# edshkim98/LocalDiffusion-Hallucination

Hardware: AMD Instinct MI355X
Metric: local patches/sec (256^2, T=1000) (higher is better)
Workload: dtype bf16; 1 GPU; cfg3: 8 local patches (vertical band masks) of one 3x256x256 image per GPU, 4-stage dim-32 conditional UNet (12.1M params), DDPM T=1000, pred_x0, sigmoid schedule; patches_per_gpu=8, parallelism=patch-sharded x1, one all-gather per sample, step_graph_replay=True, whole_batch_graph_flag=False, concurrent_sub_batches=2, weight_split_levels=0

## Files before the change

include/localdiff_hip.h:

```cpp
#ifndef LOCALDIFF_HIP_H
#define LOCALDIFF_HIP_H

#include <stddef.h>
#include <stdint.h>

#ifdef __cplusplus
extern "C" {
#endif

#define LD_OK 0
#define LD_EINVAL (-1)
#define LD_EHIP (-2)
#define LD_ETIMEOUT (-3)

#define LD_F32 0
#define LD_BF16 1
#define LD_F16 2

#define LD_STAT_STRIPES 16

#define LD_ACT_NONE 0
#define LD_ACT_SILU 1
#define LD_ACT_RELU 2

// ... 125 lines not shown

int ld_linattn_kmax(const void* qkv, uint32_t* kmax_enc, int B, int n, int heads, int dim_head,
                    int dtype, void* stream);
int ld_linattn_ctx(const void* qkv, const uint32_t* kmax_enc, float* ctx_part,
                   int B, int n, int heads, int dim_head, int nchunks, int dtype, void* stream);
int ld_linattn_ctx_reduce(const float* ctx_part, int nchunks, float* ctxn, int B, int heads,
                          int dim_head, void* stream);
int ld_linattn_fold(const float* ctxn, const float* w_out ,
                    void* w_packed , int B, int C, int heads, int dim_head,
                    int perm, int dtype, void* stream);
int ld_linattn_ctxfold(const float* ctx_part, int nchunks, const float* w_out ,
                       void* w_packed , int B, int C, int heads, int dim_head,
                       int perm, int dtype, void* stream);
int ld_linattn_kvctx(const void* x, const void* wkv_packed, const float* kshift, float* ctx_part, int B,
                     int n, int C, int heads, int dim_head, int nchunks, int dtype, void* stream);
int ld_linattn_out(const void* x, const void* wq_packed, const float* qshift, const void* mfold,
                   const float* bias, const float* g2, void* out, int B, int n, int C, float q_scale,
                   int dtype, void* stream);
int ld_linattn_kvctx_terms(const void* x, const void* wkv_packed, const float* kshift, float* ctx_part, int B, int n, int C,
                           int heads, int dim_head, int nchunks, int dtype, int weight_terms, void* stream);
int ld_linattn_out_terms(const void* x, const void* wq_packed, const float* qshift, const void* mfold, const float* bias,
                         const float* g2, void* out, int B, int n, int C, float q_scale, int dtype, int weight_terms,
                         void* stream);
size_t ld_linattn_ctx_part_floats(int B, int heads, int dim_head, int nchunks);

int ld_attention(const void* qkv, void* out, int B, int n, int heads, int dim_head, int dtype,
                 void* stream);

int ld_time_mlp(const int32_t* times, int n, const float* freqs, int dim, const float* w1,
                const float* b1, const float* w2, const float* b2, int time_dim, float* temb,
                void* stream);
int ld_time_mlp_fourier(const int32_t* times, int n, const float* weights, int learned_dim, const float* w1,
                        const float* b1, const float* w2, const float* b2, int time_dim, float* temb, void* stream);
int ld_film(const float* temb, int n, int time_dim, const float* w, const float* b, int two_c,
            float* film, void* stream);

int ld_final_conv(const void* x, const float* w , const float* b, float* out_nchw,
                  int B, int H, int W, int Cin, int Cout, int dtype, void* stream);

int ld_final_step(const void* x, const float* w, const float* b, float* model_out, float* x_t, float* x0_out,
                  const float* sched, const int32_t* t_ptr, float lo, float hi, int objective, uint64_t seed,
                  int64_t noise_stream, int B, int H, int W, int Cin, int Cout, int dtype, void* stream);


int ld_final_step_at(const void* x, const float* w, const float* b, float* model_out, float* x_t, float* x0_out,
                     const float* sched, const int32_t* t_ptr, float lo, float hi, int objective, uint64_t seed,
// ... 141 lines not shown
```

localdiffusion-hallucination_amd/_cabi.py:

```python
import ctypes as C
import os

from .tuning import lib_override_path

_HERE = os.path.dirname(os.path.abspath(__file__))

LIB_PATH = lib_override_path() or os.path.join(_HERE, "csrc", "liblocaldiff_hip.so")

LD_F32, LD_BF16, LD_F16 = 0, 1, 2
ACT_NONE, ACT_SILU, ACT_RELU = 0, 1, 2
EPI_PLAIN, EPI_QKV_LINEAR, EPI_QKV_FULL, EPI_RMS_RES, EPI_RES, EPI_GN_TAIL = 0, 1, 2, 3, 4, 5
OBJ = {"pred_x0": 0, "pred_noise": 1, "pred_v": 2}
SCHED_COLS = 8
STAT_STRIPES = 16
COUNTER_CONV3X3_C32, COUNTER_CONV3X3_GENERIC, COUNTER_CONV3X3_S32 = 0, 1, 2
SEG_SRC_PLAIN, SEG_SRC_POOL, SEG_SRC_CAT_D2S = 0, 1, 2

vp, i32, i64, u64, f32 = C.c_void_p, C.c_int32, C.c_int64, C.c_uint64, C.c_float


class Src(C.Structure):
    _fields_ = [("data", vp), ("C", i32), ("pix_stride", i32), ("upsample", i32), ("gn_stats", vp),
                ("gn_gamma", vp), ("gn_beta", vp), ("gn_groups", i32), ("act", i32), ("film", vp),
                ("film_tstride", i32), ("film_bstride", i32)]
# ... 57 lines not shown
    "ld_tuning_name": (C.c_char_p, [C.c_int]),
    "ld_range_push": (C.c_int, [C.c_char_p]),
    "ld_range_pop": (C.c_int, []),
    "ld_conv3x3": (C.c_int, [C.POINTER(Conv3x3Args), vp]),
    "ld_conv1x1": (C.c_int, [C.POINTER(Conv1x1Args), vp]),
    "ld_pack_conv_weight": (C.c_int, [vp, vp, vp, C.c_int, C.c_int, C.c_int, C.c_int, C.c_int, vp]),
    "ld_pack_conv_weight_terms": (C.c_int, [vp, vp, vp, C.c_int, C.c_int, C.c_int, C.c_int, C.c_int, C.c_int, vp]),
    "ld_conv_image": (C.c_int, [vp, vp, vp, vp, vp, C.c_int, C.c_int, C.c_int, C.c_int, C.c_int,
                                C.c_int, C.c_int, vp]),
    "ld_stem_packed_bytes": (C.c_size_t, []),
    "ld_pack_stem_weight": (C.c_int, [vp, vp, C.c_int, vp]),
    "ld_conv_stem": (C.c_int, [vp, vp, vp, vp, C.c_int, C.c_int, C.c_int, C.c_int, C.c_int, vp]),
    "ld_conv_stem_begin": (C.c_int, [vp, vp, vp, vp, C.c_int, C.c_int, C.c_int, C.c_int, C.c_int, C.POINTER(StepBeginArgs), vp]),
    "ld_gn_apply": (C.c_int, [C.POINTER(GnApplyArgs), vp]),
    "ld_linattn_kmax": (C.c_int, [vp, vp, C.c_int, C.c_int, C.c_int, C.c_int, C.c_int, vp]),
    "ld_linattn_ctx": (C.c_int, [vp, vp, vp, C.c_int, C.c_int, C.c_int, C.c_int, C.c_int, C.c_int, vp]),
    "ld_linattn_ctx_reduce": (C.c_int, [vp, C.c_int, vp, C.c_int, C.c_int, C.c_int, vp]),
    "ld_linattn_fold": (C.c_int, [vp, vp, vp, C.c_int, C.c_int, C.c_int, C.c_int, C.c_int, C.c_int, vp]),
    "ld_linattn_ctxfold": (C.c_int, [vp, C.c_int, vp, vp, C.c_int, C.c_int, C.c_int, C.c_int, C.c_int, C.c_int, vp]),
    "ld_linattn_kvctx": (C.c_int, [vp, vp, vp, vp, C.c_int, C.c_int, C.c_int, C.c_int, C.c_int, C.c_int, C.c_int, vp]),
    "ld_linattn_out": (C.c_int, [vp, vp, vp, vp, vp, vp, vp, C.c_int, C.c_int, C.c_int, f32, C.c_int, vp]),
    "ld_linattn_kvctx_terms": (C.c_int, [vp, vp, vp, vp, C.c_int, C.c_int, C.c_int, C.c_int, C.c_int, C.c_int, C.c_int, C.c_int, vp]),
    "ld_linattn_out_terms": (C.c_int, [vp, vp, vp, vp, vp, vp, vp, C.c_int, C.c_int, C.c_int, f32, C.c_int, C.c_int, vp]),
    "ld_linattn_ctx_part_floats": (C.c_size_t, [C.c_int, C.c_int, C.c_int, C.c_int]),
    "ld_attention": (C.c_int, [vp, vp, C.c_int, C.c_int, C.c_int, C.c_int, C.c_int, vp]),
    "ld_time_mlp": (C.c_int, [vp, C.c_int, vp, C.c_int, vp, vp, vp, vp, C.c_int, vp, vp]),
    "ld_time_mlp_fourier": (C.c_int, [vp, C.c_int, vp, C.c_int, vp, vp, vp, vp, C.c_int, vp, vp]),
    "ld_film": (C.c_int, [vp, C.c_int, C.c_int, vp, vp, C.c_int, vp, vp]),
    "ld_final_conv": (C.c_int, [vp, vp, vp, vp, C.c_int, C.c_int, C.c_int, C.c_int, C.c_int, C.c_int, vp]),
    "ld_final_step": (C.c_int, [vp, vp, vp, vp, vp, vp, vp, vp, f32, f32, C.c_int, u64, i64, C.c_int, C.c_int, C.c_int,
                                C.c_int, C.c_int, C.c_int, vp]),
    "ld_final_step_at": (C.c_int, [vp, vp, vp, vp, vp, vp, vp, vp, f32, f32, C.c_int, u64, i64, i64, i64, vp, C.c_int,
                                   C.c_int, C.c_int, C.c_int, C.c_int, C.c_int, vp]),
    "ld_timing_begin": (C.c_int, [C.c_int]),
    "ld_timing_count": (C.c_int, []),
    "ld_timing_end": (C.c_int, [vp, C.c_int, vp]),
    "ld_timing_end_abs": (C.c_int, [vp, vp, C.c_int, vp]),
    "ld_randn": (C.c_int, [vp, i64, u64, i64, i64, vp, vp]),
    "ld_randn_at": (C.c_int, [vp, i64, i64, u64, i64, i64, vp, vp]),
    "ld_step_add": (C.c_int, [vp, C.c_int, vp]),
    "ld_step_begin": (C.c_int, [vp, C.c_size_t, vp, C.c_size_t, vp, C.c_int, vp, vp, vp]),
    "ld_step_begin_film": (C.c_int, [vp, C.c_size_t, vp, C.c_size_t, vp, C.c_int, vp, vp, vp, C.c_int, vp, vp]),
    "ld_ddim_step_at": (C.c_int, [vp, vp, vp, vp, vp, vp, f32, f32, C.c_int, i64, vp]),
    "ld_ddpm_step": (C.c_int, [vp, vp, vp, vp, vp, vp, vp, f32, f32, C.c_int, i64, vp]),
    "ld_posterior_step": (C.c_int, [vp, vp, vp, vp, vp, vp, i64, vp]),
    "ld_ddim_step": (C.c_int, [vp, vp, vp, vp, f32, f32, f32, f32, f32, f32, f32, f32, f32, C.c_int,
# ... 95 lines not shown
```

localdiffusion-hallucination_amd/csrc/linattn_fused.hip:

```cpp
#include "common.hip.h"
#include <stdlib.h>

typedef __attribute__((ext_vector_type(4))) short s16x4;

namespace {
constexpr int CTX_STRIDE = 32 * 32 + 64;
constexpr int KTN = 256;
constexpr int PROW = 96;

__device__ __forceinline__ uint2 tr8(const char* p) {
  s16x4 v = __builtin_amdgcn_ds_read_tr16_b64_v4i16((__attribute__((address_space(3))) s16x4*)(const_cast<char*>(p)));
  return __builtin_bit_cast(uint2, v);
}

struct KvCtxArgs {
  const void* x;
  const uint4* wkv;
  float* ctx_part;
  int n, C, heads, nchunks;
  const float* kshift;
  int wsplit;
};
#define KVCTX_PARAMS const void* x_, const uint4* wkv_, float* ctx_part_, int n_, int C_, int heads_, int nchunks_, const float* kshift_, int wsplit_
#define KVCTX_ARGS(a) (a).x, (a).wkv, (a).ctx_part, (a).n, (a).C, (a).heads, (a).nchunks, (a).kshift, (a).wsplit
// ... 137 lines not shown
        }
    }
  }
  float* dst = a.ctx_part + (((size_t)b * a.heads + h) * a.nchunks + ck) * CTX_STRIDE;
#pragma unroll
  for (int r = 0; r < 4; ++r) store_f32_out(&dst[(dt * 16 + kq * 4 + r) * 32 + et * 16 + li], cacc[r]);
  __syncthreads();
  float* s_z = reinterpret_cast<float*>(s_p);
#pragma unroll
  for (int m = 0; m < 2; ++m)
#pragma unroll
    for (int r = 0; r < 4; ++r) {
      const float z = wave16_sum(zs[m][r]);
      if (li == 0) s_z[wv * 32 + 16 * m + 4 * kq + r] = z;
    }
  __syncthreads();
  if (tid < 32) {
    store_f32_out(&dst[1024 + tid], s_z[tid] + s_z[32 + tid] + s_z[64 + tid] + s_z[96 + tid]);
    store_f32_out(&dst[1056 + tid], fmaxf(fmaxf(s_m[tid], s_m[32 + tid]), fmaxf(s_m[64 + tid], s_m[96 + tid])));
  }
}


template <typename T, int NCH, bool SINGLE, int WS = 0>
__global__ __launch_bounds__(256) void kvctx_wph_kernel(KVCTX_PARAMS) {
  const KvCtxArgs a{x_, wkv_, ctx_part_, n_, C_, heads_, nchunks_, kshift_, wsplit_};
  constexpr int NCW = NCH << WS;
  constexpr int PLANE = KTN * 16;
  extern __shared__ __attribute__((aligned(16))) char smem[];
  char* s_x = smem;
  float* s_rinv = reinterpret_cast<float*>(s_x + NCH * 4 * PLANE);
  const int ck = blockIdx.x, b = blockIdx.y;
  const int tid = threadIdx.x, lane = tid & 63, wv = tid >> 6, li = lane & 15, kq = lane >> 4;
  const int h = wv;
  const int n = a.n, C = a.C;
  const int npc = (n + a.nchunks - 1) / a.nchunks;
  const int lo = ck * npc, hi = min(n, lo + npc);
  uint4 A[4][NCW];
#pragma unroll
  for (int c = 0; c < NCW; ++c)
#pragma unroll
    for (int m = 0; m < 4; ++m) A[m][c] = a.wkv[(((size_t)h * NCW + c) * 4 + m) * 64 + lane];
  float cmax[2], mloc[2], zs[2];
#pragma unroll
  for (int m = 0; m < 2; ++m) { cmax[m] = -INFINITY; mloc[m] = 0.f; zs[m] = 0.f; }
  f32x4 cacc[2][2];
#pragma unroll
  for (int i = 0; i < 2; ++i)
#pragma unroll
    for (int j = 0; j < 2; ++j) cacc[i][j] = f32x4{0.f, 0.f, 0.f, 0.f};
  const T* xb = reinterpret_cast<const T*>(a.x) + (size_t)b * n * C;

  uint4 xr[NCH][4];
  auto issue = [&](int p0) {
#pragma unroll
    for (int c = 0; c < NCH; ++c)
#pragma unroll
      for (int it = 0; it < 4; ++it) {
        const int p = p0 + (it * 4 + wv) * 16 + li;
        xr[c][it] = make_uint4(0u, 0u, 0u, 0u);
        if (p < hi) xr[c][it] = *reinterpret_cast<const uint4*>(xb + (size_t)p * C + c * 32 + kq * 8);
      }
  };
  issue(lo);
  constexpr int first_pass = SINGLE ? 1 : 0;
  if (SINGLE) {
#pragma unroll
    for (int m = 0; m < 2; ++m) mloc[m] = a.kshift[h * 32 + 16 * m + li];
  }
  constexpr float LOG2E = 1.4426950408889634f;
  float m2[2];
#pragma unroll
  for (int m = 0; m < 2; ++m) m2[m] = mloc[m] * LOG2E - DT<T>::pshift;
  for (int pass = first_pass; pass < 2; ++pass) {
    for (int p0 = lo; p0 < hi; p0 += KTN) {
      __syncthreads();
      float rs[4] = {0.f, 0.f, 0.f, 0.f};
#pragma unroll
      for (int c = 0; c < NCH; ++c)
#pragma unroll
        for (int it = 0; it < 4; ++it) {
          const int qq = (it * 4 + wv) * 16 + li;
          const uint4 raw = xr[c][it];
          float v[8];
          unpack16<T>(raw, v);
#pragma unroll
          for (int e = 0; e < 8; ++e) rs[it] = fmaf(v[e], v[e], rs[it]);
          *reinterpret_cast<uint4*>(s_x + (c * 4 + kq) * PLANE + qq * 16) = raw;
        }
#pragma unroll
      for (int it = 0; it < 4; ++it) {
        float r = rs[it];
        r = kq4_sum(r);
        if (kq == 0) s_rinv[(it * 4 + wv) * 16 + li] = rms_rinv<false>(r);
      }
      __syncthreads();
      {
        const int nxt = p0 + KTN;
        if (nxt < hi) issue(nxt);
// ... 69 lines not shown
        }
      }
    }
    if (!SINGLE && pass == 0) {
#pragma unroll
      for (int m = 0; m < 2; ++m) { mloc[m] = kq4_max(cmax[m]); m2[m] = mloc[m] * LOG2E - DT<T>::pshift; }
    }
  }
  float* dst = a.ctx_part + (((size_t)b * a.heads + h) * a.nchunks + ck) * CTX_STRIDE;
#pragma unroll
  for (int dt = 0; dt < 2; ++dt)
#pragma unroll
    for (int et = 0; et < 2; ++et)
#pragma unroll
      for (int r = 0; r < 4; ++r) store_f32_out(&dst[(dt * 16 + kq * 4 + r) * 32 + et * 16 + li], cacc[dt][et][r]);
#pragma unroll
  for (int m = 0; m < 2; ++m) {
    const float z = kq4_sum(zs[m]);
    if (kq == 0) {
      store_f32_out(&dst[1024 + 16 * m + li], z);
      store_f32_out(&dst[1056 + 16 * m + li], mloc[m]);
    }
  }
}

constexpr int LINOUT_TPB = 1;

struct LinOutArgs {
  const void* x;
  const uint4* wq;
  const uint4* mfold;
  const float* bias;
  const float* g2;
  void* out;
  int n, C;
  float q_scale;
  const float* qshift;
  int wsplit;
};
#define LINOUT_PARAMS const void* x_, const uint4* wq_, const uint4* mfold_, const float* bias_, const float* g2_, const float* qshift_, \
                      int n_, int C_, void* out_, float q_scale_, int wsplit_
#define LINOUT_ARGS(a) (a).x, (a).wq, (a).mfold, (a).bias, (a).g2, (a).qshift, (a).n, (a).C, (a).out, (a).q_scale, (a).wsplit

template <typename T, int NCH, int WS = 0>
__global__ __launch_bounds__(256) void linout_kernel(LINOUT_PARAMS) {
  const LinOutArgs a{x_, wq_, mfold_, bias_, g2_, out_, n_, C_, q_scale_, qshift_, wsplit_};
// ... 184 lines not shown
      if (kshift) LD_LAUNCH((kvctx_wph_kernel<T, 4, true>), grid2, dim3(256), lds2, st, KVCTX_ARGS(a));
      else LD_LAUNCH((kvctx_wph_kernel<T, 4, false>), grid2, dim3(256), lds2, st, KVCTX_ARGS(a));
    }
    LD_LAUNCH_CHECK("linattn_kvctx(wave-per-head)");
    return LD_OK;
  }
  LD_REQUIRE(!a.wsplit, "ld_linattn_kvctx: two-term weights need heads == 4 (the wave-per-head kernel)");
  dim3 grid(nchunks, heads, B);
  const size_t lds = (size_t)nch * 4 * KTN * 16 + 2 * KTN * PROW + KTN * sizeof(float) + 128 * sizeof(float);
  if (nch == 1) {
    LD_LAUNCH((kvctx_kernel<T, 1>), grid, dim3(256), lds, st, KVCTX_ARGS(a));
  } else if (nch == 2) {
    LD_HIP(ld_allow_lds((kvctx_kernel<T, 2>), lds));
    LD_LAUNCH((kvctx_kernel<T, 2>), grid, dim3(256), lds, st, KVCTX_ARGS(a));
  } else {
    LD_HIP(ld_allow_lds((kvctx_kernel<T, 4>), lds));
    LD_LAUNCH((kvctx_kernel<T, 4>), grid, dim3(256), lds, st, KVCTX_ARGS(a));
  }
  LD_LAUNCH_CHECK("linattn_kvctx");
  return LD_OK;
}

template <typename T>
int linout_launch(const LinOutArgs& a, int B, hipStream_t st) {
  const int n = a.n, nch = a.C / 32;
  dim3 grid((n + 128 * LINOUT_TPB - 1) / (128 * LINOUT_TPB), B);
  const size_t lds = (size_t)nch * 4 * 128 * 16 + ((size_t)nch << a.wsplit) * 8 * 1024 + (size_t)4 * 2 * nch * 1024 + 128 * sizeof(float);
  if (a.wsplit) {
    LD_REQUIRE(nch <= 2, "ld_linattn_out: two-term weights are built for C = 32 / 64 (got %d)", a.C);
    if (nch == 1) LD_LAUNCH((linout_kernel<T, 1, 1>), grid, dim3(256), lds, st, LINOUT_ARGS(a));
    else LD_LAUNCH((linout_kernel<T, 2, 1>), grid, dim3(256), lds, st, LINOUT_ARGS(a));
  } else if (nch == 1) {
    LD_LAUNCH((linout_kernel<T, 1>), grid, dim3(256), lds, st, LINOUT_ARGS(a));
  } else if (nch == 2) {
    LD_LAUNCH((linout_kernel<T, 2>), grid, dim3(256), lds, st, LINOUT_ARGS(a));
  } else {
    LD_HIP(ld_allow_lds((linout_kernel<T, 4>), lds));
    LD_LAUNCH((linout_kernel<T, 4>), grid, dim3(256), lds, st, LINOUT_ARGS(a));
  }
  LD_LAUNCH_CHECK("linattn_out");
  return LD_OK;
}
}

extern "C" int ld_linattn_kvctx(const void* x, const void* wkv_packed, const float* kshift, float* ctx_part, int B,
                                int n, int C, int heads, int dim_head, int nchunks, int dtype, void* stream) {
  return ld_linattn_kvctx_terms(x, wkv_packed, kshift, ctx_part, B, n, C, heads, dim_head, nchunks, dtype, 1, stream);
}

extern "C" int ld_linattn_kvctx_terms(const void* x, const void* wkv_packed, const float* kshift, float* ctx_part, int B,
                                      int n, int C, int heads, int dim_head, int nchunks, int dtype, int weight_terms,
                                      void* stream) {
  LD_REQUIRE(weight_terms == 1 || weight_terms == 2, "ld_linattn_kvctx: weight_terms %d", weight_terms);
  LD_REQUIRE(x && wkv_packed && ctx_part && B > 0 && n > 0 && nchunks > 0, "ld_linattn_kvctx: bad args");
  LD_REQUIRE(ld_dtype_16(dtype), "ld_linattn_kvctx: 16-bit storage only (fp32 uses the unfused path)");
  LD_REQUIRE(dim_head == 32 && (C == 32 || C == 64 || C == 128), "ld_linattn_kvctx: dim_head 32, C in {32,64,128}");
  LD_REQUIRE(kshift == nullptr || heads == 4, "ld_linattn_kvctx: the single-sweep mode (kshift) needs heads == 4");
  KvCtxArgs a{x, (const uint4*)wkv_packed, ctx_part, n, C, heads, nchunks, kshift, weight_terms == 2 ? 1 : 0};
  hipStream_t st = reinterpret_cast<hipStream_t>(stream);
  return LD_DISPATCH16(dtype, kvctx_launch<T>(a, B, st));
}

extern "C" int ld_linattn_out(const void* x, const void* wq_packed, const float* qshift, const void* mfold,
                              const float* bias, const float* g2, void* out, int B, int n, int C, float q_scale,
                              int dtype, void* stream) {
  return ld_linattn_out_terms(x, wq_packed, qshift, mfold, bias, g2, out, B, n, C, q_scale, dtype, 1, stream);
}

extern "C" int ld_linattn_out_terms(const void* x, const void* wq_packed, const float* qshift, const void* mfold,
                                    const float* bias, const float* g2, void* out, int B, int n, int C, float q_scale,
                                    int dtype, int weight_terms, void* stream) {
  LD_REQUIRE(weight_terms == 1 || weight_terms == 2, "ld_linattn_out: weight_terms %d", weight_terms);
  LD_REQUIRE(x && wq_packed && mfold && bias && g2 && out && B > 0 && n > 0, "ld_linattn_out: bad args");
  LD_REQUIRE(ld_dtype_16(dtype), "ld_linattn_out: 16-bit storage only (fp32 uses the unfused path)");
  LD_REQUIRE(C == 32 || C == 64 || C == 128, "ld_linattn_out: C in {32,64,128}");
  LinOutArgs a{x, (const uint4*)wq_packed, (const uint4*)mfold, bias, g2, out, n, C, q_scale, qshift, weight_terms == 2 ? 1 : 0};
  return LD_DISPATCH16(dtype, linout_launch<T>(a, B, reinterpret_cast<hipStream_t>(stream)));
}
```

localdiffusion-hallucination_amd/unet.py:

```python
import ctypes as C
import math

import numpy as np
import torch
from torch import nn

from . import _cabi as cabi
from .pool import check_declared, intervals_from_declared, peak_live, place_intervals
from .tuning import Tuning
from .weights import UnetConfig, unet_param_shapes

_TORCH_DT = {"fp32": torch.float32, "bf16": torch.bfloat16, "fp16": torch.float16}
_LOWP = ("bf16", "fp16")


def _register(root: nn.Module, dotted: str, tensor: torch.Tensor):
    parts = dotted.split(".")
    mod = root
    for name in parts[:-1]:
        if name not in mod._modules:
            mod.add_module(name, nn.Module())
        mod = mod._modules[name]
    mod.register_parameter(parts[-1], nn.Parameter(tensor, requires_grad=False))

# ... 191 lines not shown
                    part = part.contiguous()
                    out = torch.empty(part.numel(), dtype=tdt, device=dev)
                    cabi.check(lib.ld_pack_conv_weight(part.data_ptr(), None, out.data_ptr(), part.shape[0], part.shape[1],
                                                       k, 0, dt, st), "pack " + nm + tag)
                    P["w"][nm + tag] = out
                    P.setdefault("keep", []).append(part)
        if self.compute_dtype in _LOWP and self.cfg.init_dim == 32:
            wi = sd["init_conv.weight"].contiguous()
            stem = torch.empty(int(lib.ld_stem_packed_bytes()), dtype=torch.uint8, device=dev)
            cabi.check(lib.ld_pack_stem_weight(wi.data_ptr(), stem.data_ptr(), wi.shape[1], st), "pack init_conv")
            P["stem"] = stem
            P.setdefault("keep", []).append(wi)
        for name, w in sd.items():
            if name.endswith(".to_out.1.g"):
                g = w.flatten()
                P["g2"][name] = (g * math.sqrt(g.numel())).contiguous()
        half = self.cfg.dim // 2
        step = math.log(self.theta) / (half - 1)
        P["freqs"] = torch.exp(torch.arange(half) * -step).to(dev)
        torch.cuda.current_stream().synchronize()
        self._packed, self._packed_key = P, key
        return P

    def plan(self, B, H, W, table_T=None, instance=0):
        f = self.downsample_factor
        assert H % f == 0 and W % f == 0, \
            f"your input dimensions {(H, W)} need to be divisible by {f}, given the unet"
        tn = self.tuning
        key = (B, H, W, table_T, self.compute_dtype, instance, self.weight_split_levels,
               tn.separate_act, tn.sep_act_max_px, tn.sep_act_min_c, tn.fusion_fold, tn.side_res_conv, tn.side_res_conv_max_px, tn.side_res_conv_px, tn.fused_step_begin, tn.linattn_chunk_px, tn.buffer_reuse, tn.recompute_stem, tn.pool_by_size, tn.pool_verify)
        if key not in self._plans:
            self._plans[key] = _Plan(self, B, H, W, table_T)
        return self._plans[key]

    @torch.no_grad()
    def forward(self, x, cond_img, time, x_self_cond=None):
        B, _, H, W = x.shape
        if self.self_condition:
            c = self.cfg.channels
            raise RuntimeError(f"Given groups=1, weight of size [{self.cfg.init_dim}, {c}, 7, 7], expected input[{B}, {2 * c}, {H}, {W}] to have "
                               f"{c} channels, but got {2 * c} channels instead (self_condition=True: ddpm.py:406-413)")
        p = self.plan(B, H, W)
        st = torch.cuda.current_stream().cuda_stream
        p.x_in.copy_(x.to(torch.float32))
        p.cond_in.copy_(cond_img.to(torch.float32))
        p.times.copy_(time.to(torch.int32))
        p.run_time(st)
        p.run_cond(st)
        p.run_main(st)
        return p.model_out.clone()


class _Plan:

    def __init__(self, net: Unet, B, H, W, table_T=None):
        self.net, self.B, self.H, self.W, self.table_T = net, B, H, W, table_T
        self.lib = cabi.lib()
        self.dev = net.device
        self.dt = cabi.dtype_code(net.compute_dtype)
        self.tdt = _TORCH_DT[net.compute_dtype]
        self.esize = 4 if self.dt == cabi.LD_F32 else 2
        self.P = net.packed()
        self.tn = net.tuning
        self.f32 = self.P["f32"]
        cfg = net.cfg
        self.cfg = cfg
        self.keep = []
        self._track = None
        self.named = {}
        self.meta = {}
        self.decl = {}
        self.live_out = []
        self.ops_time, self.ops_cond, self.ops_main = [], [], []
        self.nslot = 0
        self.stats = torch.zeros(160, B, cabi.STAT_STRIPES, 16, 2, dtype=torch.float64, device=self.dev)
        self.cond_slots = 16
        self.kmax_arena = torch.zeros(8, B, cabi.STAT_STRIPES, cfg.hidden, dtype=torch.int32, device=self.dev)
        self._kmax_cursor = 0
        self.x_in = torch.zeros(B, cfg.channels, H, W, dtype=torch.float32, device=self.dev)
# ... 342 lines not shown
        if cfg.learned_sinusoidal_dim:
            wts = f["time_mlp.0.weights"]
            self.ops_time.append(lambda st: cabi.check(lib.ld_time_mlp_fourier(
                times.data_ptr(), n, wts.data_ptr(), cfg.learned_sinusoidal_dim, f["time_mlp.1.weight"].data_ptr(),
                f["time_mlp.1.bias"].data_ptr(), f["time_mlp.3.weight"].data_ptr(), f["time_mlp.3.bias"].data_ptr(),
                td, self.temb.data_ptr(), st), "time_mlp (learned Fourier features)"))
        else:
            self.ops_time.append(lambda st: cabi.check(lib.ld_time_mlp(
                times.data_ptr(), n, freqs.data_ptr(), cfg.dim, f["time_mlp.1.weight"].data_ptr(),
                f["time_mlp.1.bias"].data_ptr(), f["time_mlp.3.weight"].data_ptr(), f["time_mlp.3.bias"].data_ptr(),
                td, self.temb.data_ptr(), st), "time_mlp"))
        for name in f:
            if name.endswith(".mlp.1.weight") and not name.startswith("conv_fusion"):
                p = name[:-len(".mlp.1.weight")]
                two_c = f[name].shape[0]
                film = torch.zeros(n, two_c, dtype=torch.float32, device=self.dev)
                self.films[p] = film
                self._film_off[id(film)] = self.film_row
                self.film_row += two_c
                w, b = f[name], f[p + ".mlp.1.bias"]
                self.ops_time.append(lambda st, w=w, b=b, film=film, two_c=two_c: cabi.check(lib.ld_film(
                    self.temb.data_ptr(), n, td, w.data_ptr(), b.data_ptr(), two_c, film.data_ptr(), st), "film"))

    def resnet_block(self, ops, p, srcs_fn, cin_total, cout, h, w, res_tensor=None):
        f, G = self.f32, self.cfg.resnet_block_groups
        s1, s2 = self.slot(), self.slot()
        wres = self.P["w"].get(p + ".res_conv.weight")
        side = None
        px_ok = (h * w in self.tn.side_res_conv_px) if self.tn.side_res_conv_px is not None else h * w <= self.tn.side_res_conv_max_px
        if (wres is not None and self.tn.side_res_conv and self.dt != cabi.LD_F32 and px_ok and self.net.weight_split_levels == 0
                and wres.data_ptr() not in self.P["terms2"] and self.P["w"][p + ".block1.proj.weight"].data_ptr() not in self.P["terms2"]):
            side = (wres, f[p + ".res_conv.bias"])
        rc = None
        if side is not None:
            raw1, rc = self.conv3(ops, srcs_fn(), p + ".block1.proj", cout, h, w, stats=s1, groups=G, side=side)
        else:
            raw1 = self.conv3(ops, srcs_fn(), p + ".block1.proj", cout, h, w, stats=s1, groups=G)
        film = self.films.get(p)
        n1 = self.src(raw1, cout, gn=(s1, f[p + ".block1.norm.weight"], f[p + ".block1.norm.bias"], G),
                      act=cabi.ACT_SILU, film=film)
        if self._separate_act(h * w, cout):
            act1 = self.gn_apply(ops, n1, None, h, w, cout)
            n1 = self.src(act1, cout)
        raw2 = self.conv3(ops, [n1], p + ".block2.proj", cout, h, w, stats=s2, groups=G)
        n2 = self.src(raw2, cout, gn=(s2, f[p + ".block2.norm.weight"], f[p + ".block2.norm.bias"], G),
                      act=cabi.ACT_SILU)
        if rc is not None:
            out = self.gn_apply(ops, n2, self.src(rc, cout), h, w, cout)
        elif (p + ".res_conv.weight") in f:
            out = self.conv1(ops, srcs_fn(), self.P["w"][p + ".res_conv.weight"], cout, h, w,
                             bias=f[p + ".res_conv.bias"], epi=cabi.EPI_GN_TAIL, gn_tail=n2, what="res_conv+tail " + p)
        else:
            assert res_tensor is not None and cin_total == cout
            out = self.gn_apply(ops, n2, self.src(res_tensor, cout), h, w, cout)
        self.named[p] = out
        return out

    def fusion_block_folded(self, ops, x, c, h, w):
        f, G, p = self.f32, self.cfg.resnet_block_groups, "conv_fusion"
        p1, p2, zero = self.fusion_const
        s1, s2 = self.slot(), self.slot()
        raw1 = self.conv3(ops, [self.src(x, c)], p + ".block1.proj", c, h, w, stats=s1, groups=G,
                          weight=self.P["w"][p + ".block1.proj.weight#x"], bias=zero, addend=p1)
        n1 = self.src(raw1, c, gn=(s1, f[p + ".block1.norm.weight"], f[p + ".block1.norm.bias"], G),
                      act=cabi.ACT_SILU, film=self.films.get(p))
        if self._separate_act(h * w, c):
            n1 = self.src(self.gn_apply(ops, n1, None, h, w, c), c)
        raw2 = self.conv3(ops, [n1], p + ".block2.proj", c, h, w, stats=s2, groups=G)
        n2 = self.src(raw2, c, gn=(s2, f[p + ".block2.norm.weight"], f[p + ".block2.norm.bias"], G), act=cabi.ACT_SILU)
        out = self.conv1(ops, [self.src(x, c)], self.P["w"][p + ".res_conv.weight#x"], c, h, w, bias=None,
                         epi=cabi.EPI_GN_TAIL, gn_tail=n2, residual=p2, what="res_conv+tail " + p)
        self.named[p] = out
        return out

    def linear_attention_fused(self, ops, p, x, c, h, w):
        f, cfg, lib = self.f32, self.cfg, self.lib
        n, hid, B, heads, dt, es = h * w, cfg.hidden, self.B, cfg.attn_heads, self.dt, self.esize
        rule = self.tn.chunk_rule(B)
        chunk_px = rule[0] if n >= 65536 else (rule[1] if n >= 16384 else rule[2])
        nchunks = max(1, min(128, n // chunk_px)) if heads == 4 else max(1, min(32, n // 256))
        if heads == 4 and self.tn.linattn_chunk_px is None:
            while B * nchunks < 512 and nchunks < 512 and n // (2 * nchunks) >= 256:
                nchunks *= 2
        ctx = self._tracked(torch.empty(int(lib.ld_linattn_ctx_part_floats(B, heads, 32, nchunks)), dtype=torch.float32, device=self.dev))
        wfold = self._tracked(torch.empty(B, c * hid, dtype=self.tdt, device=self.dev))
        wout = f[p + ".to_out.0.weight"].reshape(c, hid).contiguous()
        wq, wkv = self.P["wq"][p], self.P["wkv"][p]
        kshift = self.P["kshift"].get(p) if heads == 4 else None
        ksp = kshift.data_ptr() if kshift is not None else None
        qshift = self.P["qshift"].get(p) if heads == 4 else None
        qsp = qshift.data_ptr() if qshift is not None else None
        bias, g2 = f[p + ".to_out.0.bias"], self.P["g2"][p + ".to_out.1.g"]
        out = self.buf(h, w, c)
        self.keep += [ctx, wfold, wout, wq, wkv, kshift, qshift, bias, g2, out, x]
        npx = B * n
        terms = self.P.get("attn_terms", {}).get(p, 1)
        self._raw(ops, lambda st: cabi.check(lib.ld_linattn_kvctx_terms(x.data_ptr(), wkv.data_ptr(), ksp, ctx.data_ptr(), B, n, c,
                                                                        heads, 32, nchunks, dt, terms, st), "linattn_kvctx"),
                  "linattn_kvctx", nbytes=npx * c * es, flops=2 * npx * c * 2 * hid * (1 if kshift is not None else 2) + 2 * npx * hid * 32,
                  reads=[x], writes=[ctx])
        self._raw(ops, lambda st: cabi.check(lib.ld_linattn_ctxfold(ctx.data_ptr(), nchunks, wout.data_ptr(), wfold.data_ptr(), B, c,
                                                                    heads, 32, 1, dt, st), "linattn_ctxfold"),
                  "linattn_ctxfold", nbytes=B * c * hid * es, flops=2 * B * c * hid * 32, reads=[ctx], writes=[wfold])
        scale = cfg.attn_dim_head ** -0.5
        self._raw(ops, lambda st: cabi.check(lib.ld_linattn_out_terms(x.data_ptr(), wq.data_ptr(), qsp, wfold.data_ptr(), bias.data_ptr(),
                                                                      g2.data_ptr(), out.data_ptr(), B, n, c, scale, dt, terms, st),
                                             "linattn_out"),
                  "linattn_out", nbytes=2 * npx * c * es, flops=2 * npx * hid * c * 2, reads=[x, wfold], writes=[out])
        return out

    def linear_attention(self, ops, p, x, c, h, w):
        if self.dt != cabi.LD_F32 and c in (32, 64, 128) and p in self.P["wq"]:
            return self.linear_attention_fused(ops, p, x, c, h, w)
        f, cfg, lib = self.f32, self.cfg, self.lib
        n, hid, B = h * w, cfg.hidden, self.B
        kmax = self.kmax_arena[self._kmax_cursor]
        self._kmax_cursor += 1
        qkv = self.conv1(ops, [self.src(x, c)], self.P["w"][p + ".to_qkv.weight"], 3 * hid, h, w,
                         epi=cabi.EPI_QKV_LINEAR, rms_in=1, what="to_qkv " + p, kmax_out=kmax)
        nchunks = max(1, min(32, n // 256))
        ctx = torch.empty(int(lib.ld_linattn_ctx_part_floats(B, cfg.attn_heads, 32, nchunks)),
                          dtype=torch.float32, device=self.dev)
        wfold = torch.empty(B, c * hid, dtype=self.tdt, device=self.dev)
# ... 8 lines not shown
                                                                    B, c, heads, 32, 0, dt, st), "linattn_ctxfold"),
                  "linattn_ctxfold", nbytes=B * c * hid * es, flops=2 * B * c * hid * 32, reads=[ctx], writes=[wfold])
        q = self.src(qkv, hid, stride=3 * hid)
        return self.conv1(ops, [q], wfold, c, h, w, bias=f[p + ".to_out.0.bias"], epi=cabi.EPI_RMS_RES,
                          bstride=c * hid * self.esize, g2=self.P["g2"][p + ".to_out.1.g"], residual=x,
                          what="lin to_out " + p)

    def full_attention(self, ops, p, x, c, h, w):
        f, cfg, lib = self.f32, self.cfg, self.lib
        n, hid, B = h * w, cfg.hidden, self.B
        qkv = self.conv1(ops, [self.src(x, c)], self.P["w"][p + ".to_qkv.weight"], 3 * hid, h, w,
                         epi=cabi.EPI_QKV_FULL, rms_in=1, what="to_qkv " + p)
        att = self.buf(h, w, hid)
        dt, heads = self.dt, cfg.attn_heads
        self.keep += [qkv, att]
        self._raw(ops, lambda st: cabi.check(lib.ld_attention(qkv.data_ptr(), att.data_ptr(), B, n, heads, 32, dt, st),
                                             "attention"),
                  "attention", nbytes=4 * B * n * hid * self.esize, flops=4 * B * n * n * hid, reads=[qkv], writes=[att])
        return self.conv1(ops, [self.src(att, hid)], self.P["w"][p + ".to_out.weight"], c, h, w,
                          bias=f[p + ".to_out.bias"], epi=cabi.EPI_RES, residual=x, what="full to_out " + p)

    def attention(self, ops, p, x, c, h, w, full):
        out = (self.full_attention if full else self.linear_attention)(ops, p, x, c, h, w)
        self.named[p] = out
        return out

    def _basic_block(self, ops, p, x, cin, cmid, cout, h, w, pool, image=False):
        f, lib, G = self.f32, self.lib, 16
        s1, s2, s3 = self.slot(), self.slot(), self.slot()

        def image_conv(wname, c_out, stats):
            out = self.buf(h, w, c_out)
            wt, bs = f[wname + ".weight"], f[wname + ".bias"]
            B, dt = self.B, self.dt
            self.keep += [out, wt, bs]
            ops.append(lambda st: cabi.check(lib.ld_conv_image(
                self.cond_in.data_ptr(), wt.data_ptr(), bs.data_ptr(), out.data_ptr(), stats.data_ptr(), G,
                B, cin, h, w, 3, dt, st), "conv_image " + wname))
            return out

        if image:
            a1 = image_conv(p + ".convblock.0", cmid, s1)
            idr = image_conv(p + ".identity.0", cout, s3)
        else:
            a1 = self.conv3(ops, [self.src(x, cin)], p + ".convblock.0", cmid, h, w, stats=s1, groups=G)
            idr = self.conv3(ops, [self.src(x, cin)], p + ".identity.0", cout, h, w, stats=s3, groups=G)
# ... 28 lines not shown
                za, ba, zb, bb = self._begin_args
                rows, row_floats, cur = self._film_args
                g = cabi.StepBeginArgs(za, ba, zb, bb, self._t_dev_ptr, int(delta), idx_ptr, t_table, rows, row_floats, cur)
                cabi.check(lib.ld_conv_stem_begin(self.x_in.data_ptr(), wstem.data_ptr(), bi.data_ptr(), r.data_ptr(), B, cfg.channels,
                                                  H, W, self.dt, C.byref(g), st), "init_conv + step_begin")
            self._stem_begin = stem_begin
            self._raw(ops, lambda st: cabi.check(lib.ld_conv_stem(
                self.x_in.data_ptr(), wstem.data_ptr(), bi.data_ptr(), r.data_ptr(), B, cfg.channels, H, W, self.dt, st),
                "init_conv"), "conv_image7x7",
                nbytes=B * H * W * (4 * cfg.channels + self.esize * cfg.init_dim), flops=2 * 49 * cfg.channels * cfg.init_dim * B * H * W, writes=[r])
        else:
            self._raw(ops, lambda st: cabi.check(lib.ld_conv_image(
                self.x_in.data_ptr(), wi.data_ptr(), bi.data_ptr(), r.data_ptr(), None, 1, B, cfg.channels, H, W, 7,
                self.dt, st), "init_conv"), "conv_image7x7",
                nbytes=B * H * W * (4 * cfg.channels + self.esize * cfg.init_dim), flops=2 * 49 * cfg.channels * cfg.init_dim * B * H * W, writes=[r])
        self.named["init_conv"] = r
        x, c, h, w = r, cfg.init_dim, H, W
        skips = []
        io, n = cfg.in_out, len(cfg.in_out)
        for i, (cin, cout) in enumerate(io):
            p = f"downs.{i}"
            x = self.resnet_block(ops, p + ".0", lambda x=x, c=c: [self.src(x, c)], c, c, h, w, res_tensor=x)
            skips.append((x, c))
            x = self.resnet_block(ops, p + ".1", lambda x=x, c=c: [self.src(x, c)], c, c, h, w, res_tensor=x)
            x = self.attention(ops, p + ".2", x, c, h, w, cfg.full_attn[i])
            skips.append((x, c))
            if i < n - 1:
                h, w = h // 2, w // 2
                x = self.conv1(ops, [self.src(x, c)], self.P["w"][p + ".3.1.weight"], cout, h, w,
                               bias=f[p + ".3.1.bias"], unshuffle=1, what="downsample " + p)
            else:
                x = self.conv3(ops, [self.src(x, c)], p + ".3", cout, h, w)
            self.named[p + ".3"] = x
            c = cout
        x = self.resnet_block(ops, "mid_block1", lambda x=x, c=c: [self.src(x, c)], c, c, h, w, res_tensor=x)
        x = self.attention(ops, "mid_attn", x, c, h, w, True)
        x = self.resnet_block(ops, "mid_block2", lambda x=x, c=c: [self.src(x, c)], c, c, h, w, res_tensor=x)
        feat = self.cond_feat
        if self.fusion_const is not None:
            x = self.fusion_block_folded(ops, x, c, h, w)
        else:
            x = self.resnet_block(ops, "conv_fusion", lambda x=x, c=c: [self.src(x, c), self.src(feat, c)], 2 * c, c, h, w)
        for j, ((cin, cout), full) in enumerate(zip(reversed(io), reversed(cfg.full_attn))):
            p = f"ups.{j}"
            for k in (0, 1):
                sk, sc = skips.pop()
                x = self.resnet_block(ops, f"{p}.{k}", lambda x=x, c=c, sk=sk, sc=sc: [self.src(x, c), self.src(sk, sc)],
                                      c + sc, cout, h, w)
                c = cout
            x = self.attention(ops, p + ".2", x, c, h, w, full)
            if j < n - 1:
                h, w = h * 2, w * 2
                x = self.conv3(ops, [self.src(x, c, ups=1)], p + ".3.1", cin, h, w)
            else:
                x = self.conv3(ops, [self.src(x, c)], p + ".3", cin, h, w)
            self.named[p + ".3"] = x
            c = cin
        if self.tn.recompute_stem and self._track is not None and self.dt != cabi.LD_F32 and cfg.init_dim == 32:
            r2 = self.buf(H, W, cfg.init_dim)
            wstem2 = self.P["stem"]
            self._raw(ops, lambda st, r2=r2: cabi.check(lib.ld_conv_stem(
                self.x_in.data_ptr(), wstem2.data_ptr(), bi.data_ptr(), r2.data_ptr(), B, cfg.channels, H, W, self.dt, st),
                "init_conv (again)"), "conv_image7x7",
                nbytes=B * H * W * (4 * cfg.channels + self.esize * cfg.init_dim), flops=2 * 49 * cfg.channels * cfg.init_dim * B * H * W, writes=[r2])
            r_cat = r2
        else:
            r_cat = r
        x = self.resnet_block(ops, "final_res_block", lambda x=x, c=c, r_cat=r_cat: [self.src(x, c), self.src(r_cat, cfg.init_dim)],
                              c + cfg.init_dim, cfg.dim, h, w)
        wf = f["final_conv.weight"].reshape(cfg.out_dim, cfg.dim).contiguous()
        bf = f["final_conv.bias"]
# ... 98 lines not shown
```

Baseline: 6.724 patches/s.

## Fuse ResnetBlock GroupNorm-SiLU-residual tail into linear-attention kv/context kernel

Adds a kvctx_tail kernel that applies the block2 GroupNorm affine, SiLU and residual add to the raw conv output on load, writes the block output, and runs the linear-attention key/value context pass in the same sweep. The planner defers the ResnetBlock tail whenever the next op is a foldable linear attention (16-bit, C 32/64, 4 heads). This drops one separate gn_apply launch and one full read of the block output per fused site. In exchange the kernel reads two inputs, computes GN coefficients per block and holds more registers, which may lower occupancy.

```diff
diff --git a/include/localdiff_hip.h b/include/localdiff_hip.h
--- a/include/localdiff_hip.h
+++ b/include/localdiff_hip.h
@@ -171,6 +171,9 @@
 int ld_linattn_out_terms(const void* x, const void* wq_packed, const float* qshift, const void* mfold, const float* bias,
                          const float* g2, void* out, int B, int n, int C, float q_scale, int dtype, int weight_terms,
                          void* stream);
+int ld_linattn_kvctx_tail(const void* raw2, const double* gn_stats, const float* gn_gamma, const float* gn_beta, int gn_groups,
+                          const void* res, void* out, const void* wkv_packed, const float* kshift, float* ctx_part, int B, int n,
+                          int C, int heads, int dim_head, int nchunks, int dtype, void* stream);
 size_t ld_linattn_ctx_part_floats(int B, int heads, int dim_head, int nchunks);
 
 int ld_attention(const void* qkv, void* out, int B, int n, int heads, int dim_head, int dtype,
diff --git a/localdiffusion-hallucination_amd/_cabi.py b/localdiffusion-hallucination_amd/_cabi.py
--- a/localdiffusion-hallucination_amd/_cabi.py
+++ b/localdiffusion-hallucination_amd/_cabi.py
@@ -103,6 +103,7 @@
     "ld_linattn_out": (C.c_int, [vp, vp, vp, vp, vp, vp, vp, C.c_int, C.c_int, C.c_int, f32, C.c_int, vp]),
     "ld_linattn_kvctx_terms": (C.c_int, [vp, vp, vp, vp, C.c_int, C.c_int, C.c_int, C.c_int, C.c_int, C.c_int, C.c_int, C.c_int, vp]),
     "ld_linattn_out_terms": (C.c_int, [vp, vp, vp, vp, vp, vp, vp, C.c_int, C.c_int, C.c_int, f32, C.c_int, C.c_int, vp]),
+    "ld_linattn_kvctx_tail": (C.c_int, [vp, vp, vp, vp, C.c_int, vp, vp, vp, vp, vp, C.c_int, C.c_int, C.c_int, C.c_int, C.c_int, C.c_int, C.c_int, vp]),
     "ld_linattn_ctx_part_floats": (C.c_size_t, [C.c_int, C.c_int, C.c_int, C.c_int]),
     "ld_attention": (C.c_int, [vp, vp, C.c_int, C.c_int, C.c_int, C.c_int, C.c_int, vp]),
     "ld_time_mlp": (C.c_int, [vp, C.c_int, vp, C.c_int, vp, vp, vp, vp, C.c_int, vp, vp]),
diff --git a/localdiffusion-hallucination_amd/csrc/linattn_fused.hip b/localdiffusion-hallucination_amd/csrc/linattn_fused.hip
--- a/localdiffusion-hallucination_amd/csrc/linattn_fused.hip
+++ b/localdiffusion-hallucination_amd/csrc/linattn_fused.hip
@@ -183,9 +183,22 @@
 }
 
 
-template <typename T, int NCH, bool SINGLE, int WS = 0>
-__global__ __launch_bounds__(256) void kvctx_wph_kernel(KVCTX_PARAMS) {
-  const KvCtxArgs a{x_, wkv_, ctx_part_, n_, C_, heads_, nchunks_, kshift_, wsplit_};
+struct KvTailHead {
+  const void* res;
+  const double* stats;
+  const float* gamma;
+  const float* beta;
+  int groups;
+};
+struct KvTailRest {
+  const float* kshift;
+  float* ctx_part;
+  void* out;
+};
+typedef const KvTailRest __attribute__((address_space(4)))* KvTailRestPtr;
+
+template <typename T, int NCH, bool SINGLE, int WS, bool TAIL>
+__device__ __forceinline__ void kvctx_wph_body(KvCtxArgs a, const KvTailHead& th, KvTailRestPtr rest) {
   constexpr int NCW = NCH << WS;
   constexpr int PLANE = KTN * 16;
   extern __shared__ __attribute__((aligned(16))) char smem[];
@@ -211,23 +224,54 @@
 #pragma unroll
     for (int j = 0; j < 2; ++j) cacc[i][j] = f32x4{0.f, 0.f, 0.f, 0.f};
   const T* xb = reinterpret_cast<const T*>(a.x) + (size_t)b * n * C;
+  const T* rb = TAIL ? reinterpret_cast<const T*>(th.res) + (size_t)b * n * C : nullptr;
 
   uint4 xr[NCH][4];
+  uint4 rr_[TAIL ? NCH : 1][4];
   auto issue = [&](int p0) {
 #pragma unroll
     for (int c = 0; c < NCH; ++c)
 #pragma unroll
       for (int it = 0; it < 4; ++it) {
         const int p = p0 + (it * 4 + wv) * 16 + li;
-        xr[c][it] = make_uint4(0u, 0u, 0u, 0u);
-        if (p < hi) xr[c][it] = *reinterpret_cast<const uint4*>(xb + (size_t)p * C + c * 32 + kq * 8);
+        if constexpr (TAIL) {
+          const size_t e = (size_t)min(p, hi - 1) * C + c * 32 + kq * 8;
+          xr[c][it] = *reinterpret_cast<const uint4*>(xb + e);
+          rr_[c][it] = *reinterpret_cast<const uint4*>(rb + e);
+        } else {
+          xr[c][it] = make_uint4(0u, 0u, 0u, 0u);
+          if (p < hi) xr[c][it] = *reinterpret_cast<const uint4*>(xb + (size_t)p * C + c * 32 + kq * 8);
+        }
       }
   };
   issue(lo);
+  constexpr int NCT = TAIL ? NCH : 1;
+  float gca[NCT][8], gsa[NCT][8];
+  T* ob = nullptr;
+  float ksh[2] = {0.f, 0.f};
+  if constexpr (TAIL) {
+    float* s_coef = s_rinv + KTN;
+    SrcDev S{};
+    S.stats = th.stats; S.gamma = th.gamma; S.beta = th.beta; S.film = nullptr;
+    S.C = C; S.ld = C; S.groups = th.groups; S.act = LD_ACT_SILU;
+    KvTailRestPtr pr = rest;
+    asm volatile("" : "+s"(pr));
+    a.kshift = pr->kshift; a.ctx_part = pr->ctx_part;
+    void* outp = pr->out;
+    build_gn_coef<DT<T>::precise>(S, b, 0, (long)n, s_coef, reinterpret_cast<double*>(s_coef + 2 * C), tid, 256, [&] {
+#pragma unroll
+      for (int m = 0; m < 2; ++m) ksh[m] = a.kshift[h * 32 + 16 * m + li];
+    });
+    ob = reinterpret_cast<T*>(outp) + (size_t)b * n * C;
+#pragma unroll
+    for (int c = 0; c < NCH; ++c)
+#pragma unroll
+      for (int e = 0; e < 8; ++e) { gca[c][e] = s_coef[c * 32 + kq * 8 + e]; gsa[c][e] = s_coef[C + c * 32 + kq * 8 + e]; }
+  }
   constexpr int first_pass = SINGLE ? 1 : 0;
   if (SINGLE) {
 #pragma unroll
-    for (int m = 0; m < 2; ++m) mloc[m] = a.kshift[h * 32 + 16 * m + li];
+    for (int m = 0; m < 2; ++m) mloc[m] = TAIL ? ksh[m] : a.kshift[h * 32 + 16 * m + li];
   }
   constexpr float LOG2E = 1.4426950408889634f;
   float m2[2];
@@ -236,6 +280,30 @@
   for (int pass = first_pass; pass < 2; ++pass) {
     for (int p0 = lo; p0 < hi; p0 += KTN) {
       __syncthreads();
+      if constexpr (TAIL) {
+#pragma unroll
+        for (int c = 0; c < NCH; ++c)
+#pragma unroll
+          for (int it = 0; it < 4; ++it) {
+            float v[8], u[8];
+            unpack16<T>(xr[c][it], v);
+            affine_act_n<DT<T>::precise, 8>(v, gca[c], gsa[c], LD_ACT_SILU);
+            unpack16<T>(rr_[c][it], u);
+#pragma unroll
+            for (int e = 0; e < 8; ++e) v[e] += u[e];
+            const unsigned keep = p0 + (it * 4 + wv) * 16 + li < hi ? ~0u : 0u;
+            const uint4 o = pack16<T>(v);
+            xr[c][it] = make_uint4(o.x & keep, o.y & keep, o.z & keep, o.w & keep);
+          }
+        __builtin_amdgcn_s_waitcnt(0x0F70);
+#pragma unroll
+        for (int c = 0; c < NCH; ++c)
+#pragma unroll
+          for (int it = 0; it < 4; ++it) {
+            const int p = p0 + (it * 4 + wv) * 16 + li;
+            if (p < hi) store16_out(ob + (size_t)p * C + c * 32 + kq * 8, xr[c][it]);
+          }
+      }
       float rs[4] = {0.f, 0.f, 0.f, 0.f};
 #pragma unroll
       for (int c = 0; c < NCH; ++c)
@@ -351,6 +419,23 @@
       store_f32_out(&dst[1056 + 16 * m + li], mloc[m]);
     }
   }
+}
+
+template <typename T, int NCH, bool SINGLE, int WS = 0>
+__global__ __launch_bounds__(256) void kvctx_wph_kernel(KVCTX_PARAMS) {
+  kvctx_wph_body<T, NCH, SINGLE, WS, false>(KvCtxArgs{x_, wkv_, ctx_part_, n_, C_, heads_, nchunks_, kshift_, wsplit_}, KvTailHead{}, nullptr);
+}
+
+template <typename T, int NCH>
+__global__ __launch_bounds__(256) void kvctx_tail_kernel(const void* raw_, const void* res_, const uint4* wkv_, const double* stats_,
+                                                         const float* gamma_, const float* beta_, int n_, int cg_, KvTailRest rest) {
+  constexpr unsigned REST_OFF = ld_kernarg_offset<const void*, const void*, const uint4*, const double*, const float*, const float*, int, int>(
+      alignof(KvTailRest));
+  static_assert(REST_OFF == 56, "kvctx_tail_kernel: leading arguments changed");
+  typedef const char __attribute__((address_space(4)))* KChar;
+  kvctx_wph_body<T, NCH, true, 0, true>(KvCtxArgs{raw_, wkv_, nullptr, n_, NCH * 32, 4, cg_ & 0xffff, nullptr, 0},
+                                        KvTailHead{res_, stats_, gamma_, beta_, cg_ >> 16},
+                                        (KvTailRestPtr)((KChar)__builtin_amdgcn_kernarg_segment_ptr() + REST_OFF));
 }
 
 constexpr int LINOUT_TPB = 1;
@@ -581,6 +666,18 @@
 }
 
 template <typename T>
+int kvctx_tail_launch(const void* raw2, const void* res, const uint4* wkv, const double* stats, const float* gamma, const float* beta,
+                      int cg, const KvTailRest& rest, int B, int n, int C, int nchunks, hipStream_t st) {
+  const int nch = C / 32;
+  const size_t lds = (size_t)nch * 4 * KTN * 16 + KTN * sizeof(float) + 2 * C * sizeof(float) + 2 * 16 * sizeof(float);
+  dim3 grid(nchunks, B);
+  if (nch == 1) LD_LAUNCH((kvctx_tail_kernel<T, 1>), grid, dim3(256), lds, st, raw2, res, wkv, stats, gamma, beta, n, cg, rest);
+  else LD_LAUNCH((kvctx_tail_kernel<T, 2>), grid, dim3(256), lds, st, raw2, res, wkv, stats, gamma, beta, n, cg, rest);
+  LD_LAUNCH_CHECK("linattn_kvctx_tail");
+  return LD_OK;
+}
+
+template <typename T>
 int linout_launch(const LinOutArgs& a, int B, hipStream_t st) {
   const int n = a.n, nch = a.C / 32;
   dim3 grid((n + 128 * LINOUT_TPB - 1) / (128 * LINOUT_TPB), B);
@@ -620,6 +717,25 @@
   return LD_DISPATCH16(dtype, kvctx_launch<T>(a, B, st));
 }
 
+extern "C" int ld_linattn_kvctx_tail(const void* raw2, const double* gn_stats, const float* gn_gamma, const float* gn_beta,
+                                     int gn_groups, const void* res, void* out, const void* wkv_packed, const float* kshift,
+                                     float* ctx_part, int B, int n, int C, int heads, int dim_head, int nchunks, int dtype,
+                                     void* stream) {
+  LD_REQUIRE(raw2 && gn_stats && gn_gamma && gn_beta && res && out && wkv_packed && kshift && ctx_part && B > 0 && n > 0,
+             "ld_linattn_kvctx_tail: bad args");
+  LD_REQUIRE(ld_dtype_16(dtype), "ld_linattn_kvctx_tail: 16-bit storage only");
+  LD_REQUIRE(heads == 4 && dim_head == 32 && (C == 32 || C == 64),
+             "ld_linattn_kvctx_tail: heads 4, dim_head 32, C in {32,64} (got %d, %d, %d)", heads, dim_head, C);
+  LD_REQUIRE(gn_groups > 0 && gn_groups <= 16 && C % gn_groups == 0, "ld_linattn_kvctx_tail: C=%d groups=%d", C, gn_groups);
+  LD_REQUIRE(nchunks > 0 && nchunks < (1 << 16), "ld_linattn_kvctx_tail: nchunks %d", nchunks);
+  LD_REQUIRE(out != raw2 && out != res, "ld_linattn_kvctx_tail: out must not alias an input");
+  const KvTailRest rest{kshift, ctx_part, out};
+  const int cg = nchunks | (gn_groups << 16);
+  hipStream_t st = reinterpret_cast<hipStream_t>(stream);
+  return LD_DISPATCH16(dtype, kvctx_tail_launch<T>(raw2, res, (const uint4*)wkv_packed, gn_stats, gn_gamma, gn_beta, cg, rest,
+                                                   B, n, C, nchunks, st));
+}
+
 extern "C" int ld_linattn_out(const void* x, const void* wq_packed, const float* qshift, const void* mfold,
                               const float* bias, const float* g2, void* out, int B, int n, int C, float q_scale,
                               int dtype, void* stream) {
diff --git a/localdiffusion-hallucination_amd/unet.py b/localdiffusion-hallucination_amd/unet.py
--- a/localdiffusion-hallucination_amd/unet.py
+++ b/localdiffusion-hallucination_amd/unet.py
@@ -237,15 +237,15 @@
         self._packed, self._packed_key = P, key
         return P
 
-    def plan(self, B, H, W, table_T=None, instance=0):
+    def plan(self, B, H, W, table_T=None, instance=0, _fold_tail=True):
         f = self.downsample_factor
         assert H % f == 0 and W % f == 0, \
             f"your input dimensions {(H, W)} need to be divisible by {f}, given the unet"
         tn = self.tuning
         key = (B, H, W, table_T, self.compute_dtype, instance, self.weight_split_levels,
-               tn.separate_act, tn.sep_act_max_px, tn.sep_act_min_c, tn.fusion_fold, tn.side_res_conv, tn.side_res_conv_max_px, tn.side_res_conv_px, tn.fused_step_begin, tn.linattn_chunk_px, tn.buffer_reuse, tn.recompute_stem, tn.pool_by_size, tn.pool_verify)
+               tn.separate_act, tn.sep_act_max_px, tn.sep_act_min_c, tn.fusion_fold, tn.side_res_conv, tn.side_res_conv_max_px, tn.side_res_conv_px, tn.fused_step_begin, tn.linattn_chunk_px, tn.buffer_reuse, tn.recompute_stem, tn.pool_by_size, tn.pool_verify, _fold_tail)
         if key not in self._plans:
-            self._plans[key] = _Plan(self, B, H, W, table_T)
+            self._plans[key] = _Plan(self, B, H, W, table_T, fold_tail=_fold_tail)
         return self._plans[key]
 
     @torch.no_grad()
@@ -268,8 +268,10 @@
 
 class _Plan:
 
-    def __init__(self, net: Unet, B, H, W, table_T=None):
+    def __init__(self, net: Unet, B, H, W, table_T=None, fold_tail=True):
         self.net, self.B, self.H, self.W, self.table_T = net, B, H, W, table_T
+        self._fold_tail = fold_tail
+        self._deferred_tail = None
         self.lib = cabi.lib()
         self.dev = net.device
         self.dt = cabi.dtype_code(net.compute_dtype)
@@ -658,7 +660,7 @@
                 self.ops_time.append(lambda st, w=w, b=b, film=film, two_c=two_c: cabi.check(lib.ld_film(
                     self.temb.data_ptr(), n, td, w.data_ptr(), b.data_ptr(), two_c, film.data_ptr(), st), "film"))
 
-    def resnet_block(self, ops, p, srcs_fn, cin_total, cout, h, w, res_tensor=None):
+    def resnet_block(self, ops, p, srcs_fn, cin_total, cout, h, w, res_tensor=None, fold=False):
         f, G = self.f32, self.cfg.resnet_block_groups
         s1, s2 = self.slot(), self.slot()
         wres = self.P["w"].get(p + ".res_conv.weight")
@@ -681,15 +683,33 @@
         raw2 = self.conv3(ops, [n1], p + ".block2.proj", cout, h, w, stats=s2, groups=G)
         n2 = self.src(raw2, cout, gn=(s2, f[p + ".block2.norm.weight"], f[p + ".block2.norm.bias"], G),
                       act=cabi.ACT_SILU)
-        if rc is not None:
+        if rc is not None and fold:
+            out = self._defer_tail(raw2, s2, p, rc, h, w, cout)
+        elif rc is not None:
             out = self.gn_apply(ops, n2, self.src(rc, cout), h, w, cout)
         elif (p + ".res_conv.weight") in f:
             out = self.conv1(ops, srcs_fn(), self.P["w"][p + ".res_conv.weight"], cout, h, w,
                              bias=f[p + ".res_conv.bias"], epi=cabi.EPI_GN_TAIL, gn_tail=n2, what="res_conv+tail " + p)
         else:
             assert res_tensor is not None and cin_total == cout
-            out = self.gn_apply(ops, n2, self.src(res_tensor, cout), h, w, cout)
+            if fold:
+                out = self._defer_tail(raw2, s2, p, res_tensor, h, w, cout)
+            else:
+                out = self.gn_apply(ops, n2, self.src(res_tensor, cout), h, w, cout)
         self.named[p] = out
+        return out
+
+    def _tail_foldable(self, pa, c, full):
+        return (self._fold_tail and not full and self.dt != cabi.LD_F32 and c in (32, 64) and pa in self.P["wq"]
+                and self.cfg.attn_heads == 4 and self.P["kshift"].get(pa) is not None
+                and self.P.get("attn_terms", {}).get(pa, 1) == 1)
+
+    def _defer_tail(self, raw2, s2, p, res, h, w, c):
+        f = self.f32
+        out = self.buf(h, w, c)
+        assert self._deferred_tail is None
+        self._deferred_tail = (out, raw2, s2, f[p + ".block2.norm.weight"], f[p + ".block2.norm.bias"],
+                               self.cfg.resnet_block_groups, res)
         return out
 
     def fusion_block_folded(self, ops, x, c, h, w):
@@ -731,10 +751,23 @@
         self.keep += [ctx, wfold, wout, wq, wkv, kshift, qshift, bias, g2, out, x]
         npx = B * n
         terms = self.P.get("attn_terms", {}).get(p, 1)
-        self._raw(ops, lambda st: cabi.check(lib.ld_linattn_kvctx_terms(x.data_ptr(), wkv.data_ptr(), ksp, ctx.data_ptr(), B, n, c,
-                                                                        heads, 32, nchunks, dt, terms, st), "linattn_kvctx"),
-                  "linattn_kvctx", nbytes=npx * c * es, flops=2 * npx * c * 2 * hid * (1 if kshift is not None else 2) + 2 * npx * hid * 32,
-                  reads=[x], writes=[ctx])
+        tail = self._deferred_tail
+        self._deferred_tail = None
+        if tail is not None:
+            assert tail[0] is x and kshift is not None and terms == 1 and heads == 4
+            _, raw2, st2, gam, bet, groups, res = tail
+            self.keep += [raw2, st2, gam, bet, res]
+            self._raw(ops, lambda st: cabi.check(lib.ld_linattn_kvctx_tail(raw2.data_ptr(), st2.data_ptr(), gam.data_ptr(), bet.data_ptr(),
+                                                                           groups, res.data_ptr(), x.data_ptr(), wkv.data_ptr(), ksp,
+                                                                           ctx.data_ptr(), B, n, c, heads, 32, nchunks, dt, st),
+                                                 "linattn_kvctx_tail"),
+                      "linattn_kvctx_tail", nbytes=3 * npx * c * es, flops=2 * npx * c * 2 * hid + 2 * npx * hid * 32,
+                      reads=[raw2, res], writes=[x, ctx])
+        else:
+            self._raw(ops, lambda st: cabi.check(lib.ld_linattn_kvctx_terms(x.data_ptr(), wkv.data_ptr(), ksp, ctx.data_ptr(), B, n, c,
+                                                                            heads, 32, nchunks, dt, terms, st), "linattn_kvctx"),
+                      "linattn_kvctx", nbytes=npx * c * es, flops=2 * npx * c * 2 * hid * (1 if kshift is not None else 2) + 2 * npx * hid * 32,
+                      reads=[x], writes=[ctx])
         self._raw(ops, lambda st: cabi.check(lib.ld_linattn_ctxfold(ctx.data_ptr(), nchunks, wout.data_ptr(), wfold.data_ptr(), B, c,
                                                                     heads, 32, 1, dt, st), "linattn_ctxfold"),
                   "linattn_ctxfold", nbytes=B * c * hid * es, flops=2 * B * c * hid * 32, reads=[ctx], writes=[wfold])
@@ -789,6 +822,7 @@
 
     def attention(self, ops, p, x, c, h, w, full):
         out = (self.full_attention if full else self.linear_attention)(ops, p, x, c, h, w)
+        assert self._deferred_tail is None, f"a deferred ResnetBlock tail was not taken by {p}"
         self.named[p] = out
         return out
 
@@ -863,7 +897,8 @@
             p = f"downs.{i}"
             x = self.resnet_block(ops, p + ".0", lambda x=x, c=c: [self.src(x, c)], c, c, h, w, res_tensor=x)
             skips.append((x, c))
-            x = self.resnet_block(ops, p + ".1", lambda x=x, c=c: [self.src(x, c)], c, c, h, w, res_tensor=x)
+            x = self.resnet_block(ops, p + ".1", lambda x=x, c=c: [self.src(x, c)], c, c, h, w, res_tensor=x,
+                                  fold=self._tail_foldable(p + ".2", c, cfg.full_attn[i]))
             x = self.attention(ops, p + ".2", x, c, h, w, cfg.full_attn[i])
             skips.append((x, c))
             if i < n - 1:
@@ -887,7 +922,7 @@
             for k in (0, 1):
                 sk, sc = skips.pop()
                 x = self.resnet_block(ops, f"{p}.{k}", lambda x=x, c=c, sk=sk, sc=sc: [self.src(x, c), self.src(sk, sc)],
-                                      c + sc, cout, h, w)
+                                      c + sc, cout, h, w, fold=k == 1 and self._tail_foldable(p + ".2", cout, full))
                 c = cout
             x = self.attention(ops, p + ".2", x, c, h, w, full)
             if j < n - 1:
```

Result: no change. 6.733 patches/s (median of 5 runs) (+0.1%).
